# vfrantc/Bayesian-Enhancement-Model

Measured on AMD Instinct MI355X. Metric: images/sec (whole node) CG_UNet N=8 Bayesian eval @256x256, higher is better.
Workload: dtype f32

## Files before the change

bayesian-enhancement-model_amd/bem/archs.py:

```python
from __future__ import annotations

import math
import os

import torch
import torch.nn as nn

from . import autograd as ag
from . import ops
from .modules import (Conv2dK, ConvT2x2, LayerNorm2d, PwConv2d, VSSBlock, _need_cuda, grad_mode, make_vss_level,
                      set_module_paths)
from .native import BemNativeError

_QD_DIR = os.path.join(os.path.dirname(os.path.dirname(os.path.abspath(__file__))), "basicsr", "QD", "checkpoints")


def _trunc_normal_(t, std=0.02):
    return nn.init.trunc_normal_(t, mean=0.0, std=std, a=-2.0, b=2.0)


def _init_weights(m):
    if isinstance(m, nn.Linear):
        _trunc_normal_(m.weight, std=0.02)
        if m.bias is not None:
            nn.init.constant_(m.bias, 0)
    elif isinstance(m, nn.LayerNorm):
        nn.init.constant_(m.weight, 1.0)
        nn.init.constant_(m.bias, 0)


def conv_down(c):
    return Conv2dK(c, c * 2, 4, 2, 1, bias=False)


class _CrossAttnParams(nn.Module):

    def __init__(self, dim):
        super().__init__()
        for n in ("q1_proj", "k2_proj", "v2_proj", "q2_proj", "k1_proj", "v1_proj", "out1", "out2"):
            setattr(self, n, nn.Conv2d(dim, dim, 1))


class Decomp(nn.Module):

    def __init__(self, model="model4", wavelet_out=True, num_filters=32):
        super().__init__()
        if model not in ("model1", "model2", "model3", "model4"):
            raise ValueError(f"Unknown decomp_model: {model}")
        self.model, self.wavelet_out = model, wavelet_out
        nf = num_filters
        self.conv_in = Conv2dK(32, nf, 3, padding=1)
        if model == "model3":
            self.down_conv = Conv2dK(nf, nf, 3, stride=2, padding=1)
            self.mid_conv = Conv2dK(nf, nf, 3, padding=1)
            self.up_conv = ConvT2x2(nf, nf)
        d = 2 if model == "model2" else 1
        self.branch_q1 = nn.Sequential(Conv2dK(nf, nf, 3, padding=1), nn.ReLU(inplace=True), Conv2dK(nf, nf, 3, padding=d, dilation=d))
        self.branch_q2 = nn.Sequential(Conv2dK(nf, nf, 3, padding=1), nn.ReLU(inplace=True), Conv2dK(nf, nf, 3, padding=d, dilation=d))
        self.cross_attn = _CrossAttnParams(nf)
        self.fuse = nn.Conv2d(nf * 2, nf, 1)
        self.conv_out = Conv2dK(nf, 32, 3, padding=1)
        self.sharpening = Conv2dK(32, 32, 3, padding=1, bias=True)
        if model == "model4" and not wavelet_out:
# ... 87 lines not shown


def _hamilton(o1, o2, train):
    if train:
        return ag.HamiltonFn.apply(o1, o2)
    B, _, H, W = o1.shape
    out8 = torch.empty(B, 8, H, W, device=o1.device, dtype=o1.dtype)
    ops.copy_channels(o1, out8, 0)
    ops.copy_channels(o2, out8, 4)
    return ops.hamilton(out8)


class _Stage2(nn.Module):

    def _setup(self, stage, num_blocks, d_state, ssm_ratio, mlp_ratio, mlp_type, decomp_model, wavelet_out):
        self.stage, self.num_levels = stage, len(num_blocks)
        if isinstance(d_state, int):
            d_state = [d_state] * self.num_levels
        if decomp_model is not None:
            self.decomp = Decomp.from_shipped(decomp_model, wavelet_out=wavelet_out)
        return lambda dim, i: make_vss_level(dim, num_blocks[i], d_state[i], ssm_ratio, mlp_ratio, mlp_type)

    def _add_encoder(self, sfx, cin, n_feat, level):
        setattr(self, "first_conv" + sfx, _first_conv(cin, n_feat))
        enc, cur = nn.ModuleList(), n_feat
        for i in range(self.num_levels - 1):
            enc.append(level(cur, i))
            cur *= 2
        setattr(self, "encoders" + sfx, enc)
        return cur

    def _add_down_layers(self, sfx, n_feat):
        setattr(self, "down_layers" + sfx, nn.ModuleList([conv_down(n_feat * (2 ** i)) for i in range(self.num_levels - 1)]))

    def _add_decoder(self, sfx, cur, n_feat, out_ch, level):
        decs = nn.ModuleList()
        for i in range(self.num_levels - 2, -1, -1):
            decs.append(_Dec({"up": ConvT2x2(cur, cur // 2), "fuse": PwConv2d(cur, cur // 2, bias=False), "block": level(cur // 2, i)}))
            cur //= 2
        setattr(self, "decoders" + sfx, decs)
        pj = Conv2dK(n_feat, out_ch, 3, 1, 1, bias=True)
        nn.init.zeros_(pj.bias)
        setattr(self, "proj" + sfx, pj)

    def _encode(self, sfx, x, **first_kw):
        f = getattr(self, "first_conv" + sfx)(x, **first_kw)
        skips = []
        for enc, down in zip(getattr(self, "encoders" + sfx), getattr(self, "down_layers" + sfx)):
            f, s = ag.fork(enc(f))
            skips.append(s)
            f = down(f)
        return f, skips

    def _decode(self, sfx, f, skips):
        for dec, skip in zip(getattr(self, "decoders" + sfx), reversed(skips)):
            f = dec["block"](dec["fuse"](dec["up"](f), x2=skip, in_mode=2))
        return getattr(self, "proj" + sfx)(f)

    def _cross_fuse(self, f1, f2):
        fa, fb = ag.fork(f1)
        f2 = self.cross_fusion_12(fa, f2)
        f2a, f2b = ag.fork(f2)
        return self.cross_fusion_21(f2a, fb), f2b

    def _attn_bottleneck(self, sfx, f, train):
        f = getattr(self, "bottleneck" + sfx)(f)
        se, sa = getattr(self, "bottleneck_se" + sfx), getattr(self, "spatial_attention" + sfx)
        return sa(se(f)) if train else sa(f, chan_scale=se.gate(f))


class _DualBranch(_Stage2):
    _wavelet, _in_ch, _out_ch = False, 4, 4

    def __init__(self, in_channels=3, out_channels=3, n_feat=40, stage=1, num_blocks=[2, 2, 2], d_state=1, ssm_ratio=1,
                 mlp_ratio=4, mlp_type="gdmlp", use_pixelshuffle=False, drop_path=0.0, use_illu=False, sam=False,
                 last_act=None, decomp_model="model1"):
        super().__init__()
        level = self._setup(stage, num_blocks, d_state, ssm_ratio, mlp_ratio, mlp_type, decomp_model, self._wavelet)
        for br in ("_Q1", "_Q2"):
            cur = self._add_encoder(br, self._in_ch, n_feat, level)
            self._add_down_layers(br, n_feat)
        self.bottleneck_fuse = PwConv2d(cur * 2, cur, bias=False)
        self.bottleneck_block = level(cur, -1)
        self.bottleneck_to_Q1 = PwConv2d(cur, cur, bias=False)
        self.bottleneck_to_Q2 = PwConv2d(cur, cur, bias=False)
        for br in ("_Q1", "_Q2"):
            self._add_decoder(br, cur, n_feat, self._out_ch, level)
        self.last_act = _check_last_act(last_act)
        self.apply(_init_weights)

    def _dual_unet(self, qs, first_kw=({}, {})):
        feats, skips = [], []
        for br, q, kw in zip(("_Q1", "_Q2"), qs, first_kw):
            f, sk = self._encode(br, q, **kw)
            feats.append(f)
            skips.append(sk)
        fused = self.bottleneck_block(self.bottleneck_fuse(feats[0], x2=feats[1], in_mode=2))
        return [self._decode(br, getattr(self, "bottleneck_to" + br)(fz), sk) for br, fz, sk in zip(("_Q1", "_Q2"), ag.fork(fused), skips)]

    def _full_res(self, qs):
        train = grad_mode(self)
        with torch.enable_grad() if train else torch.no_grad():
            return _hamilton(*self._dual_unet(qs), train)


class DecompDualBranchDDWavelet(_DualBranch):
    _wavelet, _in_ch, _out_ch = True, 32, 16

    def decompose(self, x, c0):
        return self.decomp(x, c0)

    def decompose_cond(self, conds, scale):
        return self.decomp.forward_from_dwt(ops.cond_dwt(conds, scale))

    def first_conv_image(self, d_img):
        fcs = [getattr(self, "first_conv" + br) for br in ("_Q1", "_Q2")]
        return [ops.conv2d(d_img, fc.conv_weight((0, 16)), fc.bias.detach(), pad=1, cin_slice=(16 * bi, 16)) for bi, fc in enumerate(fcs)]

    def forward_decomposed(self, d_img, d_cond, img_index=None, p_img=None):
        B, _, h, w = d_cond.shape
        spi = 1 if img_index is None else int(img_index)
        if d_img.shape[0] * spi != B:
            raise ValueError("forward_decomposed: image / sample batch mismatch")
        if not grad_mode(self):
            if p_img is None:
                p_img = self.first_conv_image(d_img)
            o1, o2 = self._dual_unet((d_cond, d_cond), [dict(cin_slice=(16 * bi, 16), w_part=(16, 16), use_bias=False, res1=p_img[bi], res1_rep=spi)
                                                        for bi in range(2)])
            return ops.iwt_hamilton(o1, o2)

        def branch_input(bi):
            q = torch.empty(B, 32, h, w, device=d_cond.device, dtype=d_cond.dtype)
            if spi == 1:
                ops.copy_channels(d_img, q, 0, src_c0=16 * bi, C=16)
            else:
                ops.copy_channels_rep(d_img, q, 0, spi, src_c0=16 * bi, C=16)
            ops.copy_channels(d_cond, q, 16, src_c0=16 * bi, C=16)
            return q
        o1, o2 = self._dual_unet(branch_input(bi) for bi in range(2))
        if o1.requires_grad or o2.requires_grad:
            return ag.IwtHamiltonFn.apply(o1, o2)
        return ops.iwt_hamilton(o1, o2)

    def forward(self, x, mask=None):
        _need_cuda(x)
        train = grad_mode(self)
        with torch.no_grad():
            x = x.contiguous()
            if x.shape[1] != 6:
                raise ValueError("DecompDualBranchDDWavelet expects 6 input channels (image || condition)")
            d_img, d_cond = self.decomp(x, 0), self.decomp(x, 3)
# ... 490 lines not shown
```

bayesian-enhancement-model_amd/bem/modules.py:

```python
from __future__ import annotations

import math
from typing import Dict, List, Optional

import torch
import torch.nn as nn

from . import autograd as ag
from . import ops
from .native import BemNativeError


def grad_mode(m: nn.Module) -> bool:
    return m.training and torch.is_grad_enabled()


def _need_cuda(x):
    if not x.is_cuda:
        raise BemNativeError("BEM modules run on the GPU through libbem_hip.so only (no CPU fallback); "
                             "move the model and input to a HIP device")


class SampleCtx:

# ... 94 lines not shown


class DwConv2d(nn.Conv2d):

    def __init__(self, ch, bias=True):
        super().__init__(ch, ch, 3, 1, 1, groups=ch, bias=bias)
        self.module_path = ""

    def dw_weights(self, B):
        return self.weight.detach(), (self.bias.detach() if self.bias is not None else None)


class Conv2dK(nn.Conv2d):

    def __init__(self, *a, **k):
        super().__init__(*a, **k)

    def conv_weight(self, part=None):
        w = self.weight
        return ops.derived(self).get(("part", part), [w], lambda: ops.ConvWeight(
            w.detach() if part is None else w.detach()[:, part[0]:part[0] + part[1]].contiguous()))

    def forward(self, x, relu=False, res1=None, res2=None, cin_slice=None, res1_rep=1, w_part=None, use_bias=True):
        _need_cuda(x)
        if grad_mode(self) and self.weight.requires_grad:
            if relu or res1 is not None or res2 is not None or w_part is not None or not use_bias:
                raise BemNativeError("Conv2dK: the training path covers the plain convolution (+ bias) only")
            return ag.Conv2dFn.apply(x, self.weight, self.bias, self, cin_slice)
        return ops.conv2d(x, self.conv_weight(w_part), self.bias.detach() if (use_bias and self.bias is not None) else None,
                          stride=self.stride[0], pad=self.padding[0], relu=relu, res1=res1, res2=res2, cin_slice=cin_slice, dilation=self.dilation[0],
                          res1_rep=res1_rep)


class ConvT2x2(nn.ConvTranspose2d):

    def __init__(self, cin, cout):
        super().__init__(cin, cout, kernel_size=2, stride=2, padding=0, output_padding=0)

    def forward(self, x):
        _need_cuda(x)
        if grad_mode(self):
            return ag.ConvT2x2Fn.apply(x, self.weight, self.bias, self)
        return self._forward_nograd(x)

    def _forward_nograd(self, x):
        co = self.out_channels

        def prep():
            w = self.weight.detach()
            w4 = w.permute(2, 3, 1, 0).reshape(4 * co, self.in_channels).contiguous()
            return ops.pack_pw_weight(w4), self.bias.detach().repeat(4).contiguous()
        Wp, b4 = ops.derived(self).get("p", [self.weight, self.bias], prep)
        return ops.pw_gemm(x, Wp, 4 * co, bias=b4, convT_Win=x.shape[3])


class _BayesBase(nn.Module):
    def _init_common(self, sigma_init, decay, bias):
        self.deterministic = False
        self.decay, self.sigma_init, self.step = decay, sigma_init, 0
        self.bias = bias
        self.module_path = ""

    def _rho_init(self):
        return math.log(math.expm1(abs(self.sigma_init)) + 1e-20)

    def _register_priors(self):
        for kind in ("weight", "bias") if self.bias else ("weight",):
            self.register_buffer(f"prior_mu_{kind}", getattr(self, f"mu_{kind}").detach().clone(), persistent=False)
            self.register_buffer(f"prior_rho_{kind}", getattr(self, f"rho_{kind}").detach().clone(), persistent=False)
        self._ws = self._bs = self._eps_w = self._eps_b = self._sample_owner = None

    def _train_sample(self):
        step = _TRAIN_STEP[0]
        if step is None:
            raise BemNativeError("Bayesian leaves: a training-mode forward runs under Network.forward, which scopes the weight sample")
        if self._sample_owner is step:
            return
        ctx = _SAMPLE_CTX[0]
        from .train import STEP_STATE
        st = STEP_STATE[0]
        decay = lambda: min(self.decay, (1 + self.step) / (10 + self.step))
        d, d_dev = decay(), (st.slot(decay) if st is not None else None)
        for kind in ("weight", "bias") if self.bias else ("weight",):
            mu, rho = getattr(self, f"mu_{kind}"), getattr(self, f"rho_{kind}")
            ops.bnn_prior_ema_(getattr(self, f"prior_mu_{kind}"), getattr(self, f"prior_rho_{kind}"), mu.detach(), rho.detach(), d, d_dev)
            if ctx.eps is not None:
                e = ctx.eps[f"{self.module_path}.{kind}"].reshape((1,) + tuple(mu.shape)).contiguous()
            else:
                e = ops.randn((1,) + tuple(mu.shape), mu.device, ctx.seed, ctx.next_stream(), ctx.epoch_dev)
                self.__dict__.setdefault("_draw_order", {})[kind] = ctx.counter - getattr(step, "counter0", 0)
            w = ops.bnn_sample(mu.detach(), rho.detach(), 1, e)[0]
            if kind == "weight":
                self._ws, self._eps_w = w, e
            else:
                self._bs, self._eps_b = w, e
        if st is None:
            self.step += 1
        else:
            st.on_advance(self._count_step)
        self._sample_owner = step
        step.leaves.append(self)

    def _count_step(self):
        self.step += 1

    def fold_sample_grads(self):
# ... 474 lines not shown
```

bayesian-enhancement-model_amd/bem/native.py:

```python
from __future__ import annotations

import ctypes
import os
from ctypes import c_double, c_float, c_int, c_int64, c_uint64, c_void_p

_HERE = os.path.dirname(os.path.abspath(__file__))
LIB_PATH = os.environ.get("BEM_HIP_LIB", os.path.join(os.path.dirname(_HERE), "lib", "libbem_hip.so"))
CSRC = os.path.join(os.path.dirname(_HERE), "csrc")


class BemNativeError(RuntimeError):
    pass


class PwArgs(ctypes.Structure):
    _fields_ = [
        ("x1", c_void_p), ("x2", c_void_p), ("C1", c_int), ("C2", c_int), ("in_mode", c_int),
        ("ln_w", c_void_p), ("ln_b", c_void_p), ("ln_eps", c_float),
        ("Wp", c_void_p), ("w_bstride", c_int64),
        ("bias", c_void_p), ("bias_bstride", c_int64),
        ("res", c_void_p),
        ("prelu", c_void_p), ("act", c_int),
        ("out", c_void_p), ("out_mode", c_int), ("Win", c_int),
        ("B", c_int), ("M", c_int), ("K", c_int), ("L", c_int),
    ]


class WgradArgs(ctypes.Structure):
    _fields_ = [
        ("dy", c_void_p), ("dy_bstride", c_int64), ("M", c_int),
        ("x1", c_void_p), ("x1_bstride", c_int64), ("C1", c_int),
        ("x2", c_void_p), ("x2_bstride", c_int64), ("C2", c_int),
        ("dw", c_void_p), ("ldw", c_int64), ("blk_rows", c_int), ("perm", c_int * 4),
        ("dbias", c_void_p),
        ("B", c_int), ("L", c_int),
    ]


P, I, I64, U64, F = c_void_p, c_int, c_int64, c_uint64, c_float

SIGNATURES = {
    "bem_selective_scan_fwd_f32": [P, P, P, P, P, P, P, P, I, I, I, I, I, I, P],
    "bem_selective_scan_fwd_in16": [P, P, P, P, P, P, P, P, I, I, I, I, I, I, I, P],
    "bem_cast16_to_f32": [P, P, ctypes.c_int64, I, P],
    "bem_cast_f32_to16": [P, P, ctypes.c_int64, I, P],
    "bem_selective_scan_bwd_ws_elems": [I, I, I, I],
    "bem_selective_scan_bwd_f32": [P] * 16 + [I, I, I, I, I, I, P],
    "bem_cross_scan_f32": [P, P, I, I, I, I, P],
    "bem_cross_merge_f32": [P, P, I, I, I, I, P],
    "bem_ss2d_scan_strided_f32": [P, P, P, P, P, P, P, P, P, P, I, I, I, I, I64, I64, P],
    "bem_ss2d_scan_rm_supported": [I, I, I],
    "bem_ss2d_scan_rm_f32": [P, P, P, P, P, P, P, P, P, I, I, I, I, I, I64, I64, P],
    "bem_pack_pw_weight_f32": [P, P, I, I, I, P],
    "bem_pw_packed_elems": [I, I],
    "bem_pw_gemm_x6_f32": [ctypes.POINTER(PwArgs), P],
    "bem_pack_pw_weight_x6": [P, P, I, I, I, P],
    "bem_pack_pw_weight_x6_strided": [P, P, I, I, I, I64, I64, I64, P],
    "bem_pack_pw_weight_x6_jobs": [P, P, I, P, P],
    "bem_pw_x6_packed_elems": [I, I],
    "bem_bnn_sample_pack_x6": [P, P, P, P, I, I, I, U64, U64, P, I, P],
    "bem_store_words": [P, P, I, P],
    "bem_bnn_ebank_sample_f32": [P, P, I, P, U64, U64, P],
    "bem_bnn_bank_sample_f32": [P, P, I, P, P, P, P, P, F, P, U64, U64, P, P],
    "bem_bnn_bank_kl_f32": [P, P, I, P, P, P, P],
    "bem_bnn_bank_kl_bwd_f32": [P, P, I, P, P, P, P],
    "bem_bnn_bank_reparam_bwd_f32": [P, P, I, P, P, P],
    "bem_row_scale_f32": [P, P, P, I, I, P],
    "bem_se_gate_f32": [P, P, P, P, I, I, I, P],
    "bem_spatial_attention_f32": [P, P, P, P, P, I, I, I, I, I, P],
    "bem_hamilton_bwd_f32": [P, P, P, I, I, I, P],
    "bem_chan_scale_f32": [P, P, I64, P, P, F, P, I, I, I64, P],
    "bem_chan_dot_f32": [P, P, P, I, I, I64, I, P],
    "bem_se_gate_bwd_f32": [P, P, P, P, P, P, P, P, I, I, I, P],
    "bem_spatial_attention_bwd_f32": [P, P, P, P, P, P, P, I, I, I, I, I, P],
    "bem_bnn_prior_ema_f32": [P, P, P, P, F, P, I64, P],
    "bem_bnn_kl_f32": [P, P, P, P, I64, P, P],
    "bem_bnn_kl_bwd_f32": [P, P, P, P, I64, P, P, P, P],
    "bem_bnn_reparam_bwd_f32": [P, P, P, P, P, I64, P],
    "bem_mask_token_f32": [P, P, P, P, I, I, I, I, P],
    "bem_mask_token_bwd_f32": [P, P, P, P, I, I, I, I, P],
    "bem_depth_to_space_f32": [P, P, I, I, I, I, P],
    "bem_prelu_f32": [P, P, P, I64, P],
    "bem_prelu_bwd_f32": [P, P, P, P, P, I64, P],
    "bem_bilinear_up_bwd_f32": [P, P, I, I, I, I, I, P],
    "bem_gdmlp_x6_f32": [P, P, P, F, P, P, P, P, P, P, I, I, I, I, I, P],
    "bem_conv3x3_x6_f32": [P, I64, P, P, P, P, P, I, I, I, I, I, I, I, P],
    "bem_conv4x4s2_x6_f32": [P, I64, P, P, P, P, P, I, I, I, I, I, I, P],
    "bem_conv4x4s2_fast_supported": [I, I, I],
    "bem_conv3x3_rows_supported": [I, I, I],
    "bem_ss2d_front_x6_f32": [P, P, P, F, P, P, P, P, P, P, P, I, I, I, I, I, P],
    "bem_conv_taps_x6_f32": [P, I64, P, P, P, P, P, I, I, I, I, I, I, I, I, I, I, P],
    "bem_dwconv3x3_f32": [P, P, I64, P, I64, P, I, I, I, I, I, P],
    "bem_conv2d_f32": [P, I64, P, P, P, P, P, I, I, I, I, I, I, I, I, I, I, I, P],
    "bem_conv2d_mfma_f32": [P, I64, P, P, P, P, P, I, I, I, I, I, I, I, I, I, I, I, P],
    "bem_quat_dwt_f32": [P, I64, P, I, I, I, P],
    "bem_cond_dwt_f32": [P, P, I, I, I, I, P],
    "bem_dwt_f32": [P, P, I, I, I, I, P],
    "bem_iwt_f32": [P, P, I, I, I, I, P],
    "bem_iwt_hamilton_f32": [P, P, P, I, I, I, P],
    "bem_hamilton_f32": [P, P, I, I, I, P],
    "bem_hamilton_full_f32": [P, P, P, I, I, I, P],
    "bem_attn_stats_f64": [P, P, P, I, I, P],
    "bem_attn_fold_f32": [P, P, P, P, P, P, I, I, P],
    "bem_transpose_planes_f32": [P, I64, P, I64, I, I, I, I, P],
    "bem_copy_channels_f32": [P, I64, P, I64, I, I, I, P],
    "bem_copy_channels_rep_f32": [P, I64, P, I64, I, I, I, I, P],
    "bem_add_channels_f32": [P, I64, P, I64, I, I, I, P],
    "bem_bilinear_up_f32": [P, I64, P, I64, I, I, I, I, I, P],
    "bem_space_to_depth_f32": [P, P, I, I, I, I, P],
    "bem_pixel_shuffle2_f32": [P, P, I, I, I, I, P],
    "bem_bnn_sample_f32": [P, P, P, P, I, I64, U64, U64, P, P],
    "bem_select_best_f32": [P, P, P, P, P, I, I, I64, P],
    "bem_ssim_f32": [P, P, P, P, I, I, I, I, P],
# ... 75 lines not shown
```

bayesian-enhancement-model_amd/bem/ops.py:

```python
from __future__ import annotations

import ctypes
import os
from typing import Optional

import torch

from . import native
from .native import PwArgs, check, lib


def _stream():
    return ctypes.c_void_p(torch.cuda.current_stream().cuda_stream)


def _p(t: Optional[torch.Tensor]):
    return ctypes.c_void_p(0 if t is None else t.data_ptr())


def _chk(t: Optional[torch.Tensor], name: str, dtype=torch.float32, optional=False):
    if t is None:
        if optional:
            return
        raise ValueError(f"{name} is required")
# ... 224 lines not shown
    for s in sp:
        L *= s
    C2 = 0
    if in_mode:
        if x2 is None or x2.shape[0] != B or tuple(x2.shape[2:]) != sp:
            raise ValueError("pw_gemm: x2 shape")
        C2 = x2.shape[1]
    K = C1 + C2 if in_mode == 2 else C1
    if in_mode == 1 and C1 != C2:
        raise ValueError("pw_gemm sum mode: channel mismatch")
    if getattr(Wp, "_bem_mk", (M, K)) != (M, K):
        raise ValueError(f"pw_gemm: weights packed for (M, K) = {Wp._bem_mk}, called with M={M} K={K}")
    if Wp.dim() != 2 or Wp.shape[1] != packed_elems(M, K, True) or Wp.shape[0] not in (1, B):
        raise ValueError(f"pw_gemm: packed weight shape {tuple(Wp.shape)} does not match M={M} K={K} B={B} (x6 format, pack_pw_weight)")
    a = PwArgs()
    a.x1, a.x2, a.C1, a.C2, a.in_mode = x1.data_ptr(), (x2.data_ptr() if x2 is not None else 0), C1, C2, in_mode
    if ln is not None:
        lw, lb = ln
        _chk(lw, "ln_w"); _chk(lb, "ln_b")
        if lw.numel() != K or lb.numel() != K:
            raise ValueError("pw_gemm: LayerNorm size != K")
        a.ln_w, a.ln_b = lw.data_ptr(), lb.data_ptr()
    a.ln_eps = ln_eps
    a.Wp, a.w_bstride = Wp.data_ptr(), (Wp.shape[1] if Wp.shape[0] > 1 else 0)
    if bias is not None:
        if bias.shape[-1] != M or (bias.dim() == 2 and bias.shape[0] not in (1, B)):
            raise ValueError("pw_gemm: bias shape")
        a.bias, a.bias_bstride = bias.data_ptr(), (M if (bias.dim() == 2 and bias.shape[0] > 1) else 0)
    if prelu is not None:
        if prelu.numel() != 1:
            raise ValueError("pw_gemm: PReLU with one slope only")
        a.prelu, a.act = prelu.data_ptr(), 1
    if convT_Win:
        if len(sp) != 2 or sp[1] != convT_Win or M % 4 or res is not None:
            raise ValueError("pw_gemm convT mode: bad arguments")
        oshape = (B, M // 4, 2 * sp[0], 2 * sp[1])
        a.out_mode, a.Win = 1, convT_Win
    else:
        oshape = (B, M) + sp
    if res is not None:
        if tuple(res.shape) != oshape:
            raise ValueError(f"pw_gemm: residual shape {tuple(res.shape)} != {oshape}")
        a.res = res.data_ptr()
    if out is None:
        out = torch.empty(oshape, device=x1.device, dtype=x1.dtype)
    elif tuple(out.shape) != oshape or not out.is_contiguous():
        raise ValueError("pw_gemm: out shape")
    a.out = out.data_ptr()
    a.B, a.M, a.K, a.L = B, M, K, L
    check(lib().bem_pw_gemm_x6_f32(ctypes.byref(a), _stream()), "pw_gemm")
    return out


def empty_padded(shape, device, pad=4):
    n = 1
    for s_ in shape:
        n *= s_
    buf = torch.empty(n + 2 * pad, device=device, dtype=torch.float32)
    return buf[pad:pad + n].view(shape)


def _chk_packed1(op, weights):
    for nm, Wp, M, K in weights:
        if Wp.dim() != 2 or Wp.shape[0] != 1 or Wp.shape[1] != packed_elems(M, K, True) or getattr(Wp, "_bem_mk", (M, K)) != (M, K):
            raise ValueError(f"{op}: {nm} {tuple(Wp.shape)} does not match M={M} K={K} (x6 format, one weight set)")


def ss2d_front_supported(C, Mx):
    return C <= 48 and C % 8 == 0 and Mx <= 32


def ss2d_front(x, ln_w, ln_b, ln_eps, Wp_in, bias_in, dww, dwb, Wp_x, Mx):
    for n_, t in (("x", x), ("ln_w", ln_w), ("ln_b", ln_b), ("Wp_in", Wp_in), ("dww", dww), ("Wp_x", Wp_x)):
        _chk(t, n_)
    _chk(bias_in, "bias_in", optional=True); _chk(dwb, "dwb", optional=True)
    B, C, H, W = x.shape
    if not ss2d_front_supported(C, Mx):
        raise ValueError(f"ss2d_front: C = {C} (<= 48, % 8) / Mx = {Mx} (<= 32) not supported")
    if ln_w.numel() != C or ln_b.numel() != C or dww.numel() != 9 * C or (dwb is not None and dwb.numel() != C) or (bias_in is not None and bias_in.numel() != C):
        raise ValueError("ss2d_front: parameter shapes")
    _chk_packed1("ss2d_front", (("Wp_in", Wp_in, C, C), ("Wp_x", Wp_x, Mx, C)))
    xc = torch.empty_like(x)
    xd = torch.empty(B, Mx, H, W, device=x.device, dtype=x.dtype)
    check(lib().bem_ss2d_front_x6_f32(_p(x), _p(ln_w), _p(ln_b), float(ln_eps), _p(Wp_in), _p(bias_in), _p(dww), _p(dwb), _p(Wp_x), _p(xc), _p(xd),
                                      B, C, Mx, H, W, _stream()), "ss2d_front")
    return xc, xd


def gate_interleave(Hd, device):
    j = torch.arange(Hd // 16, device=device)[:, None, None]
    c = torch.arange(16, device=device)[None, :, None]
    s_ = torch.arange(2, device=device)[None, None, :]
    return (s_ * Hd + 16 * j + c).reshape(-1)


def gdmlp_x6_supported(C, Hd):
    return C <= 80 and Hd % 16 == 0


def dw_gate_params10(dww, dwb, Hd):
    w = dww.reshape(2, Hd, 9).permute(1, 2, 0)
    b = torch.zeros(Hd, 1, 2, device=dww.device, dtype=dww.dtype) if dwb is None else dwb.reshape(2, Hd).t().reshape(Hd, 1, 2)
    return torch.cat([w, b], 1).contiguous()


def gdmlp_x6(x, ln_w, ln_b, ln_eps, Wp_gate, bias_gate, dw10, Wp_out, bias_out, Hd):
# ... 1134 lines not shown
    if A.dim() != 2 or A.shape[0] != 4 * C:
        raise ValueError(f"ss2d_scan_n_bwd: A {tuple(A.shape)} is not (4C, N)")
    N = A.shape[1]
    if not ss2d_scan_n_supported(N):
        raise NotImplementedError(f"ss2d_scan_n_bwd: d_state {N} outside 1..16")
    if x1.shape != x0.shape or dy0.shape != x0.shape or dy1.shape != x0.shape or xd0.shape != (B, 2, R + 2 * N, L) or xd1.shape != xd0.shape:
        raise ValueError("ss2d_scan_n_bwd: activation shapes")
    if dtw.shape != (4, C, R) or dtb.shape != (4, C) or Ds.numel() != 4 * C or dAlog.numel() != 4 * C * N or dDs.numel() != 4 * C \
            or ddtw.numel() != 4 * C * R or ddtb.numel() != 4 * C:
        raise ValueError("ss2d_scan_n_bwd: parameter shapes")
    bs = _xd_bstrides("ss2d_scan_n_bwd", xd0, xd1, B, R + 2 * N, L)
    dx0, dx1 = torch.empty_like(x0), torch.empty_like(x0)
    dxd0 = torch.empty(B, 2, R + 2 * N, L, device=x0.device, dtype=x0.dtype)
    dxd1 = torch.empty(B, 2, R + 2 * N, L, device=x0.device, dtype=x0.dtype)
    nws = int(lib().bem_ss2d_scan_n_bwd_ws_elems(B, C, L, N))
    ws = torch.empty(max(nws, 1), device=x0.device, dtype=torch.float32)
    check(lib().bem_ss2d_scan_n_bwd_f32(_p(x0), _p(x1), _p(xd0), _p(xd1), _p(dy0), _p(dy1), _p(dtw), _p(dtb), _p(A), _p(Ds), _p(dx0), _p(dx1),
                                        _p(dxd0), _p(dxd1), _p(dAlog), _p(dDs), _p(ddtw), _p(ddtb), _p(ws), ws.numel(), B, C, L, R, N,
                                        bs[0], bs[1], _stream()), "ss2d_scan_n_bwd")
    return dx0, dx1, dxd0, dxd1


def grad_sumsq(g, acc):
    _chk(g, "g"); _chk(acc, "acc", dtype=torch.float64)
    check(lib().bem_grad_sumsq_f32(_p(g), g.numel(), _p(acc), _stream()), "grad_sumsq")
    return acc


def adamw_step_(p, g, m, v, lr, betas, eps, weight_decay, step, max_norm=0.0, sumsq=None, norm_out=None, hyper=None):
    _chk(hyper, "hyper", optional=True)
    for n, t in (("p", p), ("g", g), ("m", m), ("v", v)):
        _chk(t, n)
    _chk(sumsq, "sumsq", dtype=torch.float64, optional=True); _chk(norm_out, "norm_out", optional=True)
    n = p.numel()
    if g.numel() != n or m.numel() != n or v.numel() != n:
        raise ValueError("adamw_step: buffer sizes differ")
    check(lib().bem_adamw_step_f32(_p(p), _p(g), _p(m), _p(v), n, float(lr), float(betas[0]), float(betas[1]), float(eps), float(weight_decay),
                                   int(step), float(max_norm), _p(sumsq), _p(norm_out), _p(hyper), _stream()), "adamw_step")


_PROF = None
_KEYS = {
    "pw_x6_res<3,2,1>": ("pw_gemm", "hbm", "pw_x6_res_kernel<3, 2, 1, false, true>",
                         lambda K, M, ln, L, mode: K <= 48 and L % 2 == 0 and mode != 1),
    "pw_x6_stream<2>": ("pw_gemm", "hbm", "pw_x6_stream_kernel<2, 2, false, true, false>",
                        lambda K, M, ln, L, mode: K > 48 and not ln and M > 32 and L % 2 == 0 and mode != 1),
    "pw_gemm": ("pw_gemm", "mfma", "pw_gemm* (all variants)", lambda K, M, ln, L, mode: True),
    "gdmlp_x6<3>": ("gdmlp_x6", "mfma_bf16", "gdmlp_x6_kernel<3, 2, 2, false>", lambda C: 32 < C <= 48),
    "gdmlp_x6<5>": ("gdmlp_x6", "mfma_bf16", "gdmlp_x6_kernel<5, 3, 1, false>", lambda C: 64 < C <= 80),
    "conv2d": ("conv2d", "mfma", "conv2d_kernel", None),
    "dwconv3x3": ("dwconv3x3", "hbm", "dwconv3x3_kernel", None),
    "ss2d_scan": ("ss2d_scan", "hbm", "ss2d_scan_kernel", None),
    "transpose_planes": ("transpose_planes", "hbm", "transpose_planes_kernel", None),
    "pw_wgrad": ("pw_wgrad_", "hbm", "wgrad_x6_kernel<2, 2> + wgrad_x6_reduce_kernel (1x1 weight gradients; wgrad_kernel<*> for L % 32 != 0)", None),
    "conv_wgrad": ("conv_wgrad_", "mfma", "wgrad_kernel<*> (dense conv weight gradients)", None),
    "ss2d_scan_bwd": ("ss2d_scan_bwd", "hbm", "ss2d_scan_bwd_kernel", None),
    "dwact_bwd": ("dwact_bwd", "hbm", "dwact_bwd_kernel", None),
    "ln_bwd": ("ln_bwd", "hbm", "ln_bwd_kernel", None),
}


def profile_start(key: str):
    global _PROF
    if key not in _KEYS:
        raise ValueError(f"profile_start: unknown key {key}; choose from {sorted(_KEYS)}")
    op, bound, symbol, pred = _KEYS[key]
    _PROF = {"kernel": op, "symbol": symbol, "bound": bound, "pred": pred, "events": [], "bytes": 0.0, "flops": 0.0}


def profile_stop():
    global _PROF
    p, _PROF = _PROF, None
    if p is None:
        return None
    torch.cuda.synchronize()
    ms = sum(s.elapsed_time(e) for s, e in p["events"])
    return {"kernel": p["symbol"], "bound": p["bound"], "launches": len(p["events"]), "ms": ms,
            "bytes": p["bytes"], "flops": p["flops"]}


def _timed(name, nbytes, nflops):
    if _PROF is None or _PROF["kernel"] != name:
        return None
    s = torch.cuda.Event(enable_timing=True)
    s.record()
    _PROF["bytes"] += nbytes
    _PROF["flops"] += nflops
    return s


def _timed_end(s):
    if s is not None:
        e = torch.cuda.Event(enable_timing=True)
        e.record()
        _PROF["events"].append((s, e))


def _wrap_profiled():
    global pw_gemm, conv2d, dwconv3x3, ss2d_scan, transpose_planes
    _pw, _cv, _dw, _ss, _tp = pw_gemm, conv2d, dwconv3x3, ss2d_scan, transpose_planes

    def pw_gemm_p(x1, Wp, M, **kw):
        if _PROF is None:
            return _pw(x1, Wp, M, **kw)
        B, C1 = x1.shape[0], x1.shape[1]
        L = x1[0, 0].numel()
# ... 35 lines not shown
        if _PROF is None:
            return _ss(x0, x1, xd0, xd1, dtw, dtb, A, Ds)
        s = _timed("ss2d_scan", 4.0 * (2 * x0.numel() + 2 * xd0.numel() + 2 * x0.numel()), 0.0)
        out = _ss(x0, x1, xd0, xd1, dtw, dtb, A, Ds)
        _timed_end(s)
        return out

    def transpose_planes_p(x):
        if _PROF is None:
            return _tp(x)
        s = _timed("transpose_planes", 8.0 * x.numel(), 0.0)
        out = _tp(x)
        _timed_end(s)
        return out

    pw_gemm, conv2d, dwconv3x3, ss2d_scan, transpose_planes = pw_gemm_p, conv2d_p, dwconv3x3_p, ss2d_scan_p, transpose_planes_p

    def numel(t):
        return 0 if t is None else t.numel()

    def wrap(name, cost):
        inner = globals()[name]

        def wrapped(*a, **kw):
            if _PROF is None or _PROF["kernel"] != name:
                return inner(*a, **kw)
            nb, nf = cost(*a, **kw)
            s = _timed(name, nb, nf)
            out = inner(*a, **kw)
            _timed_end(s)
            return out
        wrapped.__doc__ = inner.__doc__
        globals()[name] = wrapped

    def c_pw_wgrad(dy, x1, dw, x2=None, dbias=None, blk_rows=0, perm=None, dy_bstride=0, M=None):
        B, L = x1.shape[0], x1[0, 0].numel()
        M = dy.shape[1] if M is None else M
        K = x1.shape[1] + (0 if x2 is None else x2.shape[1])
        return 4.0 * B * L * (M + K) + 4.0 * M * K, 2.0 * M * K * B * L

    def c_conv_wgrad(dy, x, dw, dbias=None, stride=1, pad=1, cin_slice=None):
        Cout, Cin, KH, KW = dw.shape
        return 4.0 * (dy.numel() + x.shape[0] * Cin * x.shape[2] * x.shape[3]) + 4.0 * dw.numel(), 2.0 * dy.numel() * Cin * KH * KW

    def c_scan_bwd(x0, x1, xd0, xd1, dy0, dy1, *a, **kw):
        return 4.0 * (6 * x0.numel() + 4 * xd0.numel()), 0.0

    def c_dwact(t, w, bias, dout, dw, dbias, mode):
        return 4.0 * (2 * t.numel() + dout.numel()), 40.0 * t.numel()

    def c_ln(x1, dn, gamma, beta, eps, dgamma, dbeta, x2=None, dres=None, want_n=True):
        return 4.0 * x1.numel() * (3 + (x2 is not None) + (dres is not None) + bool(want_n)), 0.0

    for nm, fn in (("pw_wgrad_", c_pw_wgrad), ("conv_wgrad_", c_conv_wgrad), ("ss2d_scan_bwd", c_scan_bwd), ("dwact_bwd", c_dwact), ("ln_bwd", c_ln)):
        wrap(nm, fn)


_wrap_profiled()
```

include/bem_hip.h:

```cpp
#ifndef BEM_HIP_H
#define BEM_HIP_H

#include <stdint.h>

#ifdef __cplusplus
extern "C" {
#endif

#define BEM_OK 0
#define BEM_ERR_INVALID 1
#define BEM_ERR_LAUNCH 2

const char* bem_last_error(void);
int bem_abi_version(void);


int bem_selective_scan_fwd_f32(const float* u, const float* delta, const float* A, const float* Bm,
                               const float* Cm, const float* D, const float* delta_bias, float* out,
                               int batch, int dim, int L, int dstate, int ngroups, int delta_softplus,
                               void* stream);

int bem_selective_scan_fwd_in16(const void* u, const void* delta, const float* A, const void* Bm, const void* Cm, const float* D,
                                const float* delta_bias, float* out, int in_dtype, int batch, int dim, int L, int dstate,
                                int ngroups, int delta_softplus, void* stream);

int bem_cast16_to_f32(const void* src, float* dst, int64_t n, int dtype, void* stream);
int bem_cast_f32_to16(const float* src, void* dst, int64_t n, int dtype, void* stream);

int64_t bem_selective_scan_bwd_ws_elems(int batch, int dim, int L, int dstate);
int bem_selective_scan_bwd_f32(const float* u, const float* delta, const float* A, const float* Bm, const float* Cm,
                               const float* D, const float* delta_bias, const float* dout, float* ws, float* du,
                               float* ddelta, float* dA, float* dB, float* dC, float* dD, float* ddelta_bias,
                               int batch, int dim, int L, int dstate, int ngroups, int delta_softplus, void* stream);

int bem_cross_scan_f32(const float* x, float* xs, int B, int C, int H, int W, void* stream);
int bem_cross_merge_f32(const float* ys, float* y, int B, int C, int H, int W, void* stream);

int bem_ss2d_scan_strided_f32(const float* x0, const float* x1, const float* xd0, const float* xd1,
                              const float* dtw, const float* dtb, const float* A, const float* Ds,
                              float* y0, float* y1, int B, int C, int L, int R, int64_t xd0_bstride, int64_t xd1_bstride,
                              void* stream);

int bem_ss2d_scan_rm_supported(int H, int W, int R);
int bem_ss2d_scan_rm_f32(const float* x, const float* xd0, const float* xd1, const float* dtw, const float* dtb,
                         const float* A, const float* Ds, float* y0, float* y1, int B, int C, int H, int W, int R,
                         int64_t xd0_bstride, int64_t xd1_bstride, void* stream);

int bem_ss2d_scan_n_supported(int N);
int bem_ss2d_scan_n_f32(const float* x0, const float* x1, const float* xd0, const float* xd1, const float* dtw, const float* dtb,
                        const float* A, const float* Ds, float* y0, float* y1, int B, int C, int L, int R, int N,
                        int64_t xd0_bstride, int64_t xd1_bstride, void* stream);

typedef struct {
    const float* x1; const float* x2; int C1; int C2; int in_mode;
    const float* ln_w; const float* ln_b; float ln_eps;
    const float* Wp; int64_t w_bstride;
    const float* bias; int64_t bias_bstride;
    const float* res;
    const float* prelu; int act;
    float* out; int out_mode; int Win;
    int B; int M; int K; int L;
} bem_pw_args;
int bem_pack_pw_weight_f32(const float* W, float* Wp, int nsets, int M, int K, void* stream);
int64_t bem_pw_packed_elems(int M, int K);

int bem_pw_gemm_x6_f32(const bem_pw_args* a, void* stream);
int bem_pack_pw_weight_x6(const float* W, float* Wp, int nsets, int M, int K, void* stream);
int bem_pack_pw_weight_x6_strided(const float* W, float* Wp, int nsets, int M, int K, int64_t set_stride, int64_t row_stride,
                                  int64_t col_stride, void* stream);
int bem_pack_pw_weight_x6_jobs(const void* jobs, const void* blks, int nblk, float* arena, void* stream);
int64_t bem_pw_x6_packed_elems(int M, int K);
int bem_bnn_sample_pack_x6(const float* mu, const float* rho, const float* eps, float* Wp, int nsets, int M, int K,
                           uint64_t seed, uint64_t stream_id, const uint64_t* stream_add, int sigma_given,
                           void* stream);

int bem_dwconv3x3_f32(const float* x, const float* w, int64_t w_bstride, const float* bias,
                      int64_t bias_bstride, float* out, int B, int Cout, int H, int W, int mode, void* stream);

int bem_conv2d_f32(const float* x, int64_t x_bstride, const float* w, const float* bias, const float* res1,
                   const float* res2, float* out, int B, int Cin, int H, int W, int Cout, int KH, int KW,
                   int stride, int pad, int relu, int res1_rep, void* stream);

int bem_conv2d_mfma_f32(const float* x, int64_t x_bstride, const float* Wp, const float* bias, const float* res1,
                        const float* res2, float* out, int B, int Cin, int H, int W, int Cout, int KH, int KW,
                        int stride, int pad, int relu, int res1_rep, void* stream);

int bem_conv3x3_x6_f32(const float* x, int64_t x_bstride, const float* Wp, const float* bias, const float* res1,
                       const float* res2, float* out, int B, int Cin, int H, int W, int Cout, int relu, int res1_rep, void* stream);
int bem_conv4x4s2_fast_supported(int Cin, int H, int W);
int bem_conv3x3_rows_supported(int Cin, int H, int W);
int bem_conv4x4s2_x6_f32(const float* x, int64_t x_bstride, const float* Wp, const float* bias, const float* res1,
                         const float* res2, float* out, int B, int Cin, int H, int W, int Cout, int relu, void* stream);

int bem_conv_taps_x6_f32(const float* x, int64_t x_bstride, const float* Wp, const float* bias, const float* res1, const float* res2,
                         float* out, int B, int Cin, int H, int W, int Cout, int K, int stride, int dilation, int relu, int res1_rep,
                         void* stream);

int bem_quat_dwt_f32(const float* rgb, int64_t x_bstride, float* out, int B, int H, int W, void* stream);
int bem_cond_dwt_f32(const float* cond, float* out, int R, int H, int W, int s, void* stream);
int bem_dwt_f32(const float* x, float* out, int B, int C, int H, int W, void* stream);
int bem_iwt_f32(const float* x, float* out, int B, int C4, int H, int W, void* stream);
int bem_iwt_hamilton_f32(const float* q1w, const float* q2w, float* out, int B, int h, int w, void* stream);
int bem_hamilton_f32(const float* q, float* out, int B, int H, int W, void* stream);

int bem_hamilton_full_f32(const float* q1, const float* q2, float* out, int B, int H, int W, void* stream);

int bem_attn_stats_f64(const float* f1, const float* f2, double* stats, int B, int L, void* stream);
int bem_attn_fold_f32(const double* stats, const float* attn_w ,
                      const float* fuse_w , const float* fuse_b ,
                      float* W_out , float* bias_out , int B, int L,
                      void* stream);

int bem_transpose_planes_f32(const float* src, int64_t src_bstride, float* dst, int64_t dst_bstride,
                             int nbatch, int ppb, int H, int W, void* stream);
int bem_copy_channels_f32(const float* src, int64_t src_bstride, float* dst, int64_t dst_bstride,
                          int B, int C, int L, void* stream);
int bem_copy_channels_rep_f32(const float* src, int64_t src_bstride, float* dst, int64_t dst_bstride, int B, int C, int L, int rep,
                              void* stream);
int bem_add_channels_f32(const float* src, int64_t src_bstride, float* dst, int64_t dst_bstride,
                         int B, int C, int L, void* stream);
int bem_bilinear_up_f32(const float* src, int64_t src_bstride, float* dst, int64_t dst_bstride,
                        int B, int C, int H, int W, int s, void* stream);
int bem_space_to_depth_f32(const float* x, float* out, int B, int C, int H, int W, void* stream);
int bem_pixel_shuffle2_f32(const float* x, float* out, int B, int C, int H, int W, void* stream);

int bem_bnn_ebank_sample_f32(const void* segs, const void* blks, int nblk, float* arena, uint64_t seed, uint64_t stream_base, void* stream);

// ... 145 lines not shown
```

Measured before the change: 314.4.

## Fold decoder upsample, fuse 1x1 and bottleneck projection into one kernel

Composes the transposed 2x2 conv weights with the first half of the fuse 1x1 conv (and optionally the preceding bottleneck_to projection) into four folded matrices, computed in double on the host and cached. A new HIP kernel then computes the upsampled-and-fused output directly from the low-res feature and the skip, so the full-resolution intermediate from the transposed conv is never written or read back. Used only in no-grad mode when the fuse layer has no bias. It costs extra FLOPs (C x C/2 per output pixel instead of a smaller product on low-res), and the weight algebra in double could shift numerics slightly.

Result: faster. 318.8 (median of 6 runs) (+1.4%).

```diff
diff --git a/bayesian-enhancement-model_amd/bem/archs.py b/bayesian-enhancement-model_amd/bem/archs.py
--- a/bayesian-enhancement-model_amd/bem/archs.py
+++ b/bayesian-enhancement-model_amd/bem/archs.py
@@ -8,7 +8,7 @@
 
 from . import autograd as ag
 from . import ops
-from .modules import (Conv2dK, ConvT2x2, LayerNorm2d, PwConv2d, VSSBlock, _need_cuda, grad_mode, make_vss_level,
+from .modules import (Conv2dK, ConvT2x2, LayerNorm2d, PwConv2d, VSSBlock, _need_cuda, fold_up_fuse, grad_mode, make_vss_level,
                       set_module_paths)
 from .native import BemNativeError
 
@@ -202,9 +202,16 @@
             f = down(f)
         return f, skips
 
-    def _decode(self, sfx, f, skips):
+    def _decode(self, sfx, f, skips, pre=None):
+        folded = ops.USE_UPFUSE and not grad_mode(self)
+        if pre is not None and not (folded and pre.bias is None):
+            f, pre = pre(f), None
         for dec, skip in zip(getattr(self, "decoders" + sfx), reversed(skips)):
-            f = dec["block"](dec["fuse"](dec["up"](f), x2=skip, in_mode=2))
+            if folded and dec["fuse"].bias is None:
+                f = ops.up_fuse(f, skip, fold_up_fuse(dec["up"], dec["fuse"], pre, holder=dec))
+            else:
+                f = dec["fuse"](dec["up"](f if pre is None else pre(f)), x2=skip, in_mode=2)
+            f, pre = dec["block"](f), None
         return getattr(self, "proj" + sfx)(f)
 
     def _cross_fuse(self, f1, f2):
@@ -246,7 +253,7 @@
             feats.append(f)
             skips.append(sk)
         fused = self.bottleneck_block(self.bottleneck_fuse(feats[0], x2=feats[1], in_mode=2))
-        return [self._decode(br, getattr(self, "bottleneck_to" + br)(fz), sk) for br, fz, sk in zip(("_Q1", "_Q2"), ag.fork(fused), skips)]
+        return [self._decode(br, fz, sk, pre=getattr(self, "bottleneck_to" + br)) for br, fz, sk in zip(("_Q1", "_Q2"), ag.fork(fused), skips)]
 
     def _full_res(self, qs):
         train = grad_mode(self)
diff --git a/bayesian-enhancement-model_amd/bem/modules.py b/bayesian-enhancement-model_amd/bem/modules.py
--- a/bayesian-enhancement-model_amd/bem/modules.py
+++ b/bayesian-enhancement-model_amd/bem/modules.py
@@ -170,6 +170,32 @@
             return ops.pack_pw_weight(w4), self.bias.detach().repeat(4).contiguous()
         Wp, b4 = ops.derived(self).get("p", [self.weight, self.bias], prep)
         return ops.pw_gemm(x, Wp, 4 * co, bias=b4, convT_Win=x.shape[3])
+
+
+def compose_up_fuse(up_w, up_b, fuse_w, pre_w=None):
+    co = up_w.shape[1]
+    wf = fuse_w.double().reshape(fuse_w.shape[0], -1)
+    wf1, wf2 = wf[:, :co], wf[:, co:]
+    wc = torch.einsum("mc,kcab->abmk", wf1, up_w.double())
+    if pre_w is not None:
+        wc = wc @ pre_w.double().reshape(pre_w.shape[0], -1)
+    return wc.reshape(4, wf.shape[0], -1), wf1 @ up_b.double(), wf2
+
+
+def fold_up_fuse(up: "ConvT2x2", fuse: PwConv2d, pre: Optional[PwConv2d] = None, holder: Optional[nn.Module] = None) -> "ops.UpFuseWeights":
+    if fuse.bias is not None or (pre is not None and pre.bias is not None):
+        raise ValueError("fold_up_fuse: a fuse / pre layer with a bias is not folded")
+    c, co = up.in_channels, up.out_channels
+    if c != 2 * co or (fuse.in_channels, fuse.out_channels) != (c, co) or (pre is not None and (pre.in_channels, pre.out_channels) != (c, c)):
+        raise ValueError(f"fold_up_fuse: needs up C -> C/2, fuse C -> C/2 and pre C -> C (got up {c} -> {co}, fuse {fuse.in_channels} -> "
+                         f"{fuse.out_channels}" + (f", pre {pre.in_channels} -> {pre.out_channels})" if pre is not None else ")"))
+    srcs = [up.weight, up.bias, fuse.weight] + ([pre.weight] if pre is not None else [])
+
+    def prep():
+        wc, bc, wf2 = compose_up_fuse(up.weight.detach(), up.bias.detach(), fuse.weight.detach(), None if pre is None else pre.weight.detach())
+        return ops.UpFuseWeights(ops.pack_pw_weight(wc.float().contiguous()), ops.pack_pw_weight(wf2.float().contiguous()),
+                                 bc.float().contiguous(), c)
+    return ops.derived(up if holder is None else holder).get(("upfuse", pre is not None), srcs, prep)
 
 
 class _BayesBase(nn.Module):
diff --git a/bayesian-enhancement-model_amd/bem/native.py b/bayesian-enhancement-model_amd/bem/native.py
--- a/bayesian-enhancement-model_amd/bem/native.py
+++ b/bayesian-enhancement-model_amd/bem/native.py
@@ -59,6 +59,7 @@
     "bem_pack_pw_weight_x6_jobs": [P, P, I, P, P],
     "bem_pw_x6_packed_elems": [I, I],
     "bem_bnn_sample_pack_x6": [P, P, P, P, I, I, I, U64, U64, P, I, P],
+    "bem_upfuse_x6_f32": [P, P, P, P, P, P, I, I, I, I, P],
     "bem_store_words": [P, P, I, P],
     "bem_bnn_ebank_sample_f32": [P, P, I, P, U64, U64, P],
     "bem_bnn_bank_sample_f32": [P, P, I, P, P, P, P, P, F, P, U64, U64, P, P],
diff --git a/bayesian-enhancement-model_amd/bem/ops.py b/bayesian-enhancement-model_amd/bem/ops.py
--- a/bayesian-enhancement-model_amd/bem/ops.py
+++ b/bayesian-enhancement-model_amd/bem/ops.py
@@ -300,6 +300,36 @@
     return out
 
 
+USE_UPFUSE = True
+
+
+class UpFuseWeights:
+
+    def __init__(self, Wc, Wf2, bias, cin):
+        self.Wc, self.Wf2, self.bias, self.cin = Wc, Wf2, bias, int(cin)
+
+
+def up_fuse(f, skip, folded: UpFuseWeights):
+    _chk(f, "f"); _chk(skip, "skip"); _chk(folded.Wc, "Wc"); _chk(folded.Wf2, "Wf2"); _chk(folded.bias, "bias")
+    if f.dim() != 4:
+        raise ValueError("up_fuse: f must be (B, Cin, h, w)")
+    B, C, h, w = f.shape
+    if C != folded.cin or C < 2 or C % 2:
+        raise ValueError(f"up_fuse: f has {C} channels, the folded weights were made for {folded.cin} (even, >= 2)")
+    Co = C // 2
+    if tuple(skip.shape) != (B, Co, 2 * h, 2 * w):
+        raise ValueError(f"up_fuse: skip shape {tuple(skip.shape)} != {(B, Co, 2 * h, 2 * w)}")
+    if tuple(folded.Wc.shape) != (4, packed_elems(Co, C, True)) or getattr(folded.Wc, "_bem_mk", (Co, C)) != (Co, C):
+        raise ValueError(f"up_fuse: Wc packed shape {tuple(folded.Wc.shape)} does not match four ({Co}, {C}) matrices")
+    if tuple(folded.Wf2.shape) != (1, packed_elems(Co, Co, True)) or getattr(folded.Wf2, "_bem_mk", (Co, Co)) != (Co, Co):
+        raise ValueError(f"up_fuse: Wf2 packed shape {tuple(folded.Wf2.shape)} does not match one ({Co}, {Co}) matrix")
+    if folded.bias.numel() != Co:
+        raise ValueError("up_fuse: bias size")
+    out = torch.empty_like(skip)
+    check(lib().bem_upfuse_x6_f32(_p(f), _p(skip), _p(folded.Wc), _p(folded.Wf2), _p(folded.bias), _p(out), B, C, h, w, _stream()), "up_fuse")
+    return out
+
+
 def empty_padded(shape, device, pad=4):
     n = 1
     for s_ in shape:
@@ -1540,6 +1570,7 @@
     "dwconv3x3": ("dwconv3x3", "hbm", "dwconv3x3_kernel", None),
     "ss2d_scan": ("ss2d_scan", "hbm", "ss2d_scan_kernel", None),
     "transpose_planes": ("transpose_planes", "hbm", "transpose_planes_kernel", None),
+    "up_fuse": ("up_fuse", "hbm", "upfuse_x6_kernel<2>", None),
     "pw_wgrad": ("pw_wgrad_", "hbm", "wgrad_x6_kernel<2, 2> + wgrad_x6_reduce_kernel (1x1 weight gradients; wgrad_kernel<*> for L % 32 != 0)", None),
     "conv_wgrad": ("conv_wgrad_", "mfma", "wgrad_kernel<*> (dense conv weight gradients)", None),
     "ss2d_scan_bwd": ("ss2d_scan_bwd", "hbm", "ss2d_scan_bwd_kernel", None),
@@ -1681,7 +1712,11 @@
     def c_ln(x1, dn, gamma, beta, eps, dgamma, dbeta, x2=None, dres=None, want_n=True):
         return 4.0 * x1.numel() * (3 + (x2 is not None) + (dres is not None) + bool(want_n)), 0.0
 
-    for nm, fn in (("pw_wgrad_", c_pw_wgrad), ("conv_wgrad_", c_conv_wgrad), ("ss2d_scan_bwd", c_scan_bwd), ("dwact_bwd", c_dwact), ("ln_bwd", c_ln)):
+    def c_up_fuse(f, skip, folded):
+        Co = skip.shape[1]
+        return 4.0 * (f.numel() + 2 * skip.numel() + folded.Wc.numel() + folded.Wf2.numel()), 2.0 * skip.numel() * (f.shape[1] + Co)
+
+    for nm, fn in (("up_fuse", c_up_fuse), ("pw_wgrad_", c_pw_wgrad), ("conv_wgrad_", c_conv_wgrad), ("ss2d_scan_bwd", c_scan_bwd), ("dwact_bwd", c_dwact), ("ln_bwd", c_ln)):
         wrap(nm, fn)
 
 
diff --git a/bayesian-enhancement-model_amd/csrc/upfuse_x6.hip b/bayesian-enhancement-model_amd/csrc/upfuse_x6.hip
--- /dev/null
+++ b/bayesian-enhancement-model_amd/csrc/upfuse_x6.hip
@@ -0,0 +1,171 @@
+#include "bem_common.h"
+#include "x6_common.h"
+
+namespace {
+
+struct UfX {
+    const float* f; const float* skip; const u32x4* Wc; const u32x4* Wf2; const float* bias; float* out;
+    int C, Co, w, L;
+    int KB, KB2, MT;
+};
+
+template <int MTW>
+__global__ __launch_bounds__(256, 2) void upfuse_x6_kernel(UfX k) {
+    const int lane = threadIdx.x & 63, wave = threadIdx.x >> 6, kh = lane >> 5, n = lane & 31;
+    const int b = blockIdx.z, a = blockIdx.y & 1, mt0 = (blockIdx.y >> 1) * MTW;
+    const int p0 = (xcd_tile(blockIdx.x, gridDim.x) * 4 + wave) * 32;
+    if (p0 >= k.L) return;
+    const int p = p0 + n;
+    const bool keep = p < k.L;
+    const int pc = keep ? p : k.L - 1;
+    const int i = pc / k.w, j = pc - i * k.w;
+    const int Lo = 4 * k.L, Wo = 2 * k.w;
+    const uint32_t hi_off = (uint32_t)(2 * i) * (uint32_t)Wo + (uint32_t)(2 * j);
+    const float* fb = k.f + (int64_t)b * k.C * k.L;
+    const float* sb = k.skip + (int64_t)b * k.Co * Lo;
+    float* ob = k.out + (int64_t)b * k.Co * Lo;
+    const bool two = MTW == 2 && mt0 + 1 < k.MT;
+
+    auto load_f = [&](int kb, float (&dst)[8]) {
+#pragma unroll
+        for (int e = 0; e < 8; ++e) {
+            const int ch = 16 * kb + 8 * kh + e;
+            const float v = fb[(uint32_t)min(ch, k.C - 1) * (uint32_t)k.L + (uint32_t)pc];
+            dst[e] = v * (ch < k.C ? 1.f : 0.f);
+        }
+    };
+    auto load_s = [&](int kb, uint32_t off, float (&dst)[8][2]) {
+#pragma unroll
+        for (int e = 0; e < 8; ++e) {
+            const int ch = 16 * kb + 8 * kh + e;
+            const float2 v = *reinterpret_cast<const float2*>(sb + ((uint32_t)min(ch, k.Co - 1) * (uint32_t)Lo + off));
+            const float mk = ch < k.Co ? 1.f : 0.f;
+            dst[e][0] = v.x * mk; dst[e][1] = v.y * mk;
+        }
+    };
+    auto load_w = [&](const u32x4* set, int kbn, int kb, u32x4 (&dst)[MTW][3]) {
+#pragma unroll
+        for (int m = 0; m < MTW; ++m) {
+            const u32x4* wp = set + ((int64_t)min(mt0 + m, k.MT - 1) * kbn + min(kb, kbn - 1)) * (3 * 64) + lane;
+#pragma unroll
+            for (int li = 0; li < 3; ++li) dst[m][li] = wp[li * 64];
+        }
+    };
+    const int64_t set_stride = (int64_t)k.MT * k.KB * 3 * 64;
+
+    {
+        const uint32_t row_off = hi_off + (uint32_t)(a * Wo);
+        const int kh4 = 4 * kh;
+        f32x16 acc[MTW][2], alo[MTW][2];
+#pragma unroll
+        for (int m = 0; m < MTW; ++m)
+#pragma unroll
+            for (int t = 0; t < 2; ++t)
+#pragma unroll
+                for (int r = 0; r < 16; ++r) acc[m][t][r] = alo[m][t][r] = 0.f;
+        u32x4 wn[MTW][3];
+        {
+            float sn[8][2];
+            load_s(0, row_off, sn);
+            load_w(k.Wf2, k.KB2, 0, wn);
+            for (int kb = 0; kb < k.KB2; ++kb) {
+                u32x4 xl[2][3], wc[MTW][3];
+#pragma unroll
+                for (int t = 0; t < 2; ++t) {
+                    float v[8];
+#pragma unroll
+                    for (int e = 0; e < 8; ++e) v[e] = sn[e][t];
+                    split8(v, xl[t][0], xl[t][1], xl[t][2]);
+                }
+#pragma unroll
+                for (int m = 0; m < MTW; ++m)
+#pragma unroll
+                    for (int li = 0; li < 3; ++li) wc[m][li] = wn[m][li];
+                load_s(kb + 1, row_off, sn);
+                load_w(k.Wf2, k.KB2, kb + 1, wn);
+#pragma unroll
+                for (int m = 0; m < MTW; ++m)
+                    if (m == 0 || two) {
+#pragma unroll
+                        for (int t = 0; t < 2; ++t) mac6(wc[m], xl[t], acc[m][t], alo[m][t]);
+                    }
+            }
+        }
+        {
+            const u32x4* w0 = k.Wc + (int64_t)(2 * a) * set_stride;
+            const u32x4* w1 = w0 + set_stride;
+            float fn[8], fn2[8];
+            load_f(0, fn);
+            load_f(1, fn2);
+            load_w(w0, k.KB, 0, wn);
+            for (int kb = 0; kb < k.KB; ++kb) {
+                u32x4 xl[3], wc[MTW][3];
+                split8(fn, xl[0], xl[1], xl[2]);
+#pragma unroll
+                for (int e = 0; e < 8; ++e) fn[e] = fn2[e];
+                load_f(kb + 2, fn2);
+#pragma unroll
+                for (int m = 0; m < MTW; ++m)
+#pragma unroll
+                    for (int li = 0; li < 3; ++li) wc[m][li] = wn[m][li];
+                load_w(w1, k.KB, kb, wn);
+#pragma unroll
+                for (int m = 0; m < MTW; ++m)
+                    if (m == 0 || two) mac6(wc[m], xl, acc[m][0], alo[m][0]);
+#pragma unroll
+                for (int m = 0; m < MTW; ++m)
+#pragma unroll
+                    for (int li = 0; li < 3; ++li) wc[m][li] = wn[m][li];
+                load_w(w0, k.KB, kb + 1, wn);
+#pragma unroll
+                for (int m = 0; m < MTW; ++m)
+                    if (m == 0 || two) mac6(wc[m], xl, acc[m][1], alo[m][1]);
+            }
+        }
+        const uint32_t loff = (uint32_t)kh4 * (uint32_t)Lo + row_off;
+#pragma unroll
+        for (int m = 0; m < MTW; ++m) {
+            if (mt0 + m >= k.MT) continue;
+            const int rb = (mt0 + m) * 32;
+#pragma unroll
+            for (int g = 0; g < 4; ++g) {
+                float bv[4];
+#pragma unroll
+                for (int q = 0; q < 4; ++q)
+                    bv[q] = valu_copy(k.bias[min(rb + 8 * g + kh4 + q, k.Co - 1)]);
+#pragma unroll
+                for (int q = 0; q < 4; ++q) {
+                    const int r = 4 * g + q, urow = rb + 8 * g + q;
+                    const float o0 = acc[m][0][r] + (alo[m][0][r] + bv[q]);
+                    const float o1 = acc[m][1][r] + (alo[m][1][r] + bv[q]);
+                    if (keep && urow + kh4 < k.Co) *reinterpret_cast<float2*>(ob + (int64_t)urow * Lo + loff) = make_float2(o0, o1);
+                }
+            }
+        }
+    }
+}
+
+}
+
+extern "C" int bem_upfuse_x6_f32(const float* f, const float* skip, const float* Wc_packed, const float* Wf2_packed, const float* bias,
+                                 float* out, int B, int Cin, int h, int w, void* stream) {
+    BEM_REQUIRE(f && skip && Wc_packed && Wf2_packed && bias && out, "upfuse_x6: null tensor");
+    BEM_REQUIRE(B >= 0 && B <= 65535 && Cin >= 2 && Cin % 2 == 0 && h > 0 && w > 0, "upfuse_x6: bad shape B=%d Cin=%d h=%d w=%d", B, Cin, h, w);
+    BEM_REQUIRE((int64_t)Cin * h * w < (1ll << 29), "upfuse_x6: Cin * h * w = %lld exceeds the 32-bit lane offsets", (long long)Cin * h * w);
+    BEM_REQUIRE((((uintptr_t)Wc_packed | (uintptr_t)Wf2_packed) & 15) == 0, "upfuse_x6: packed weights must be 16-byte aligned");
+    BEM_REQUIRE((((uintptr_t)skip | (uintptr_t)out) & 7) == 0 && ((uintptr_t)f & 3) == 0, "upfuse_x6: skip / out must be 8-byte aligned");
+    if (B == 0) return BEM_OK;
+    UfX k;
+    k.f = f; k.skip = skip; k.Wc = reinterpret_cast<const u32x4*>(Wc_packed); k.Wf2 = reinterpret_cast<const u32x4*>(Wf2_packed);
+    k.bias = bias; k.out = out;
+    k.C = Cin; k.Co = Cin / 2; k.w = w; k.L = h * w;
+    k.KB = cdiv(k.C, 16); k.KB2 = cdiv(k.Co, 16); k.MT = cdiv(k.Co, 32);
+    BEM_REQUIRE(k.MT <= 65535, "upfuse_x6: Cin %d too wide", Cin);
+    hipStream_t s = (hipStream_t)stream;
+    if (k.MT == 1) {
+        upfuse_x6_kernel<1><<<dim3(cdiv(k.L, 128), 2, B), 256, 0, s>>>(k);
+    } else {
+        upfuse_x6_kernel<2><<<dim3(cdiv(k.L, 128), 2 * cdiv(k.MT, 2), B), 256, 0, s>>>(k);
+    }
+    return bem_check_launch("upfuse_x6");
+}
diff --git a/include/bem_hip.h b/include/bem_hip.h
--- a/include/bem_hip.h
+++ b/include/bem_hip.h
@@ -73,6 +73,8 @@
 int bem_bnn_sample_pack_x6(const float* mu, const float* rho, const float* eps, float* Wp, int nsets, int M, int K,
                            uint64_t seed, uint64_t stream_id, const uint64_t* stream_add, int sigma_given,
                            void* stream);
+int bem_upfuse_x6_f32(const float* f, const float* skip, const float* Wc_packed, const float* Wf2_packed, const float* bias, float* out,
+                      int B, int Cin, int h, int w, void* stream);
 
 int bem_dwconv3x3_f32(const float* x, const float* w, int64_t w_bstride, const float* bias,
                       int64_t bias_bstride, float* out, int B, int Cout, int H, int W, int mode, void* stream);
```
